# robotseu/ORB_Line_SLAM

Measured on AMD Instinct MI355X. Metric: stereo frames/s extract+match (ORB+LBD), KITTI 1242x375, higher is better.
Workload: dtype u8; 1 GPU; C3: 1242x375 stereo, 2000 ORB + 500 LBD per image, extract + stereo point/line match + f2f LBD match + SearchByBoW vs the previous frame (synthetic k=10 L=6 vocabulary, ComputeBoW included); parallelism=frame-sharded x1, distinct_pairs=512, order=shuffled, scene=default

## Files before the change

### include/orbline.h

```cpp
#ifndef ORBLINE_H
#define ORBLINE_H

#include "orbline_types.h"

#ifdef __cplusplus
extern "C" {
#endif

typedef struct olf_ctx olf_ctx;

const char* olf_last_error(void);
int olf_device_count(void);
int olf_default_params(olf_params* p);

int  olf_ctx_create(const olf_params* p, int width, int height, int max_images, olf_ctx** out);
void olf_ctx_destroy(olf_ctx* ctx);
int  olf_ctx_synchronize(olf_ctx* ctx);
int  olf_ctx_set_input_event(olf_ctx* ctx, void* hip_event);
int  olf_ctx_set_deferred_join(olf_ctx* ctx, int on);
int  olf_stereo_frames_join_dev(olf_ctx* ctx, void* stream);
int  olf_ctx_poll_status(olf_ctx* ctx);

int olf_profile_enable(olf_ctx* ctx, int on);
int olf_profile_reset(olf_ctx* ctx);
// ... 54 lines not shown
int olf_debug_status(olf_ctx* ctx, int32_t* out64);
int olf_debug_status_n(olf_ctx* ctx, int32_t* out, int n);
int olf_debug_lsd_owner(olf_ctx* ctx, int image, uint32_t* out);
int olf_debug_lsd_regions(olf_ctx* ctx, int image, int32_t* start_n, double* angle, int cap, int32_t* count);
int olf_debug_lsd_waves(olf_ctx* ctx, int waves_per_image, int rob_entries);
int olf_debug_lsd_groups(olf_ctx* ctx, int groups);
int olf_debug_lsd_scatter(olf_ctx* ctx, int on);
int olf_debug_lsd_log_cap(olf_ctx* ctx, int entries);
int olf_debug_seed_sort(olf_ctx* ctx, const uint32_t* keys, int n, int kthr, int depth_limit, uint32_t* out, int32_t* out_n);
int olf_debug_seed_sort_mode(olf_ctx* ctx, int mode);
int olf_debug_seed_sort_wide(olf_ctx* ctx, const uint64_t* keys, int n, int64_t kthr, int depth_limit, int full, uint32_t* out, int32_t* out_n);
int olf_debug_lsd_pool(olf_ctx* ctx, int pool_chunks);
int olf_debug_fdiv_sweep(olf_ctx* ctx, uint64_t seed, int blocks, int per_thread, uint64_t* mismatches);
int olf_debug_sqrtq_sweep(olf_ctx* ctx, int count, uint64_t* mismatches);
int olf_debug_align_sweep(olf_ctx* ctx, uint64_t seed, int blocks, int per_thread, uint64_t* out3);

int olf_stereo_points_dev(olf_ctx* ctx, int n_pairs, const olf_keypoint* d_kps, const uint8_t* d_desc, const int32_t* d_counts,
                          float* d_uright, float* d_depth, void* stream);
int olf_stereo_points(olf_ctx* ctx, const uint8_t* images, int n_pairs, olf_keypoint* kps, uint8_t* desc, int32_t* counts,
                      float* uright, float* depth);

int olf_match_bf_dev(olf_ctx* ctx, const uint8_t* d_descA, const int32_t* d_nA, int strideA, int a_step, const uint8_t* d_descB,
                     const int32_t* d_nB, int strideB, int b_step, int n_sets, float nnr, int best_lr, int32_t* d_m12, void* stream);
int olf_match_bf(olf_ctx* ctx, const uint8_t* descA, int nA, const uint8_t* descB, int nB, float nnr, int best_lr, int32_t* m12);
int olf_knn2(olf_ctx* ctx, const uint8_t* descQ, int nQ, const uint8_t* descT, int nT, int32_t* idx0, int32_t* dist0, int32_t* dist1);
int olf_match_candidates_dev(olf_ctx* ctx, const uint8_t* d_descQ, int nQ, const uint8_t* d_descT, int nT, const int32_t* d_cand_offsets,
                             const int32_t* d_cand_idx, uint16_t* d_dist, void* stream);
int olf_match_candidates(olf_ctx* ctx, const uint8_t* descQ, int nQ, const uint8_t* descT, int nT, const int32_t* cand_offsets,
                         const int32_t* cand_idx, uint16_t* dist);
typedef struct olf_frame_view {
// ... 149 lines not shown
```

### orb_line_slam_amd/_lib.py

```python
import ctypes as C
import os
import numpy as np

_HERE = os.path.dirname(os.path.abspath(__file__))
LIB_PATH = os.environ.get("OLF_LIB_PATH", os.path.join(_HERE, "csrc", "liborbline_hip.so"))
SYNTH_PATH = os.path.join(_HERE, "csrc", "libolf_synth.so")

OLF_OK, OLF_ERR_INVALID, OLF_ERR_CAPACITY, OLF_ERR_HIP, OLF_ERR_NODEVICE = 0, -1, -2, -3, -4
DESC_BYTES = 32

KEYPOINT_DTYPE = np.dtype([("x", "<f4"), ("y", "<f4"), ("size", "<f4"), ("angle", "<f4"), ("response", "<f4"),
                           ("octave", "<i4"), ("class_id", "<i4")])
KEYLINE_DTYPE = np.dtype([("angle", "<f4"), ("class_id", "<i4"), ("octave", "<i4"), ("pt_x", "<f4"), ("pt_y", "<f4"),
                          ("response", "<f4"), ("size", "<f4"), ("startPointX", "<f4"), ("startPointY", "<f4"),
                          ("endPointX", "<f4"), ("endPointY", "<f4"), ("sPointInOctaveX", "<f4"),
                          ("sPointInOctaveY", "<f4"), ("ePointInOctaveX", "<f4"), ("ePointInOctaveY", "<f4"),
                          ("lineLength", "<f4"), ("numOfPixels", "<i4")])
assert KEYPOINT_DTYPE.itemsize == 28 and KEYLINE_DTYPE.itemsize == 68


class OrbParams(C.Structure):
    _fields_ = [("nfeatures", C.c_int32), ("scale_factor", C.c_float), ("nlevels", C.c_int32),
                ("ini_th_fast", C.c_int32), ("min_th_fast", C.c_int32), ("conv_gauss_sum256", C.c_int32)]

# ... 144 lines not shown
        L.olf_ctx_set_input_event.argtypes = [C.c_void_p, C.c_void_p]
        L.olf_ctx_set_deferred_join.argtypes = [C.c_void_p, C.c_int]
        L.olf_stereo_frames_join_dev.argtypes = [C.c_void_p, C.c_void_p]
        L.olf_stereo_points_mask_dev.argtypes = [C.c_void_p, C.c_void_p, C.c_size_t, C.c_void_p, C.c_void_p]
        L.olf_search_by_projection_batch_dev.argtypes = [C.c_void_p, C.POINTER(TrackBatchC), C.c_int, C.c_float, C.c_void_p, C.c_int, C.c_int,
                                                         C.c_void_p, C.c_void_p, C.c_void_p, C.c_void_p]
        L.olf_unproject_stereo_dev.argtypes = [C.c_void_p, C.c_int, C.c_int, C.c_void_p, C.c_void_p, C.c_void_p] + [C.c_float] * 4 + [C.c_void_p] * 3
        L.olf_predict_scale_thresholds.argtypes = [C.c_void_p, C.c_int, C.c_void_p]
        L.olf_is_in_frustum_batch_dev.argtypes = [C.c_void_p, C.POINTER(TrackBatchC), C.c_int, C.POINTER(LocalMapC), C.c_void_p, C.c_float] + [C.c_void_p] * 5
        L.olf_search_local_map_batch_dev.argtypes = [C.c_void_p, C.POINTER(TrackBatchC), C.c_int, C.POINTER(LocalMapC), C.c_void_p, C.c_float, C.c_float,
                                                     C.c_void_p, C.c_float, C.c_void_p, C.c_void_p, C.c_void_p]
        L.olf_debug_copy_bandwidth.argtypes =[C.c_void_p, C.c_size_t, C.c_int, C.POINTER(C.c_double)]
        L.olf_debug_fdiv_sweep.argtypes = [C.c_void_p, C.c_uint64, C.c_int, C.c_int, C.POINTER(C.c_uint64)]
        L.olf_debug_sqrtq_sweep.argtypes = [C.c_void_p, C.c_int, C.POINTER(C.c_uint64)]
        L.olf_debug_align_sweep.argtypes = [C.c_void_p, C.c_uint64, C.c_int, C.c_int, C.POINTER(C.c_uint64)]
        L.olf_debug_seed_sort_wide.argtypes = [C.c_void_p, C.c_void_p, C.c_int, C.c_int64, C.c_int, C.c_int, C.c_void_p, C.POINTER(C.c_int32)]
        L.olf_distinctive_descriptors.argtypes = [C.c_void_p, C.c_void_p, C.c_void_p, C.c_int, C.c_void_p]
        L.olf_voc_create.argtypes = [C.c_int, C.c_int, C.c_int, C.c_int, C.c_int, C.c_void_p, C.c_void_p, C.c_void_p, C.c_void_p, C.POINTER(C.c_void_p)]
        L.olf_voc_load_text.argtypes = [C.c_char_p, C.POINTER(C.c_void_p)]
        L.olf_voc_destroy.argtypes = [C.c_void_p]
        L.olf_voc_destroy.restype = None
        L.olf_voc_info.argtypes = [C.c_void_p] + [C.POINTER(C.c_int)] * 6
        L.olf_bow_words_dev.argtypes = [C.c_void_p, C.c_void_p, C.c_void_p, C.c_int, C.c_int, C.c_void_p, C.c_void_p, C.c_void_p, C.c_void_p]
        L.olf_bow_assemble.argtypes = [C.c_void_p, C.c_void_p, C.c_void_p, C.c_void_p, C.c_int, C.c_void_p, C.c_void_p, C.POINTER(C.c_int), C.c_void_p,
                                       C.c_void_p, C.c_void_p, C.POINTER(C.c_int)]
        L.olf_search_by_bow_batch_dev.argtypes = [C.c_void_p, C.c_void_p, C.c_int, C.c_int, C.c_void_p, C.c_void_p, C.c_void_p, C.c_void_p, C.c_void_p, C.c_float, C.c_int, C.c_int, C.c_void_p, C.c_void_p, C.c_void_p]
        L.olf_bow_transform.argtypes = [C.c_void_p, C.c_void_p, C.c_void_p, C.c_int, C.c_int, C.c_void_p, C.c_void_p, C.POINTER(C.c_int), C.c_void_p,
                                        C.c_void_p, C.c_void_p, C.POINTER(C.c_int)]
        L.olf_profile_enable.argtypes = [C.c_void_p, C.c_int]
        L.olf_profile_reset.argtypes = [C.c_void_p]
        L.olf_profile_stage_name.restype = C.c_char_p
        L.olf_profile_stage_name.argtypes = [C.c_int]
        L.olf_profile_read.argtypes = [C.c_void_p, C.c_void_p, C.c_void_p]
        _lib = L
    return _lib


def last_error():
    return lib().olf_last_error().decode()


def device_count():
    return int(lib().olf_device_count())


def default_params():
    p = OlfParams()
    rc = lib().olf_default_params(C.byref(p))
    if rc != OLF_OK:
        raise OlfError(rc, "olf_default_params")
    return p


def check(rc, where):
    if rc != OLF_OK:
        raise OlfError(rc, where)
# ... 51 lines not shown
```

### orb_line_slam_amd/csrc/api.cpp

```cpp
#include "olf_internal.hpp"
#include "line_internal.hpp"
#include "../../include/orbline.h"
#include <map>
#include <mutex>
#include <cstring>
#include <cstddef>

namespace olf {
static thread_local std::string g_err;
void set_error(const std::string& s) { g_err = s; }
}

using namespace olf;

enum { FB_KPS, FB_DESC, FB_COUNTS, FB_URIGHT, FB_DEPTH, FB_KLS, FB_LDESC, FB_LCOUNTS, FB_LMATCHES12, FB_LDISP, FB_LLE, FB_FIELDS };
enum FieldCap { CAP_ONE, CAP_ORB, CAP_LINE };
struct FrameField { const char* name; size_t offset; bool perPair; FieldCap cap; size_t rowBytes; };
#define FIELD(f, perPair, cap, rowBytes) {#f, offsetof(olf_frame_buffers, f), perPair, cap, rowBytes}
constexpr FrameField kFrameFields[] = {
    FIELD(kps, false, CAP_ORB, sizeof(olf_keypoint)),   FIELD(desc, false, CAP_ORB, OLF_DESC_BYTES),    FIELD(counts, false, CAP_ONE, sizeof(int32_t)),
    FIELD(uright, true, CAP_ORB, sizeof(float)),        FIELD(depth, true, CAP_ORB, sizeof(float)),
    FIELD(kls, false, CAP_LINE, sizeof(olf_keyline)),   FIELD(ldesc, false, CAP_LINE, OLF_DESC_BYTES),  FIELD(lcounts, false, CAP_ONE, sizeof(int32_t)),
    FIELD(lmatches12, true, CAP_LINE, sizeof(int32_t)), FIELD(ldisp, true, CAP_LINE, 2 * sizeof(float)), FIELD(lle, true, CAP_LINE, 3 * sizeof(double))};
#undef FIELD
// ... 714 lines not shown
    return OLF_OK;
}

int olf_debug_sqrtq_sweep(olf_ctx* c, int count, uint64_t* mismatches)
{
    if (!c || !mismatches || count < 1) { set_error("olf_debug_sqrtq_sweep: bad argument"); return OLF_ERR_INVALID; }
    void* st = nullptr;
    OLF_TRY(scratch_get(c, 1, 64, &st));
    OLF_HIP_CHECK(hipMemsetAsync(st, 0, 8, c->stream));
    OLF_TRY(launch_sqrtq_sweep(count, (unsigned long long*)st, c->stream));
    OLF_HIP_CHECK(hipMemcpyAsync(mismatches, st, 8, hipMemcpyDeviceToHost, c->stream));
    OLF_HIP_CHECK(hipStreamSynchronize(c->stream));
    return OLF_OK;
}

int olf_debug_align_sweep(olf_ctx* c, uint64_t seed, int blocks, int per_thread, uint64_t* out3)
{
    if (!c || !out3 || blocks < 1 || per_thread < 1) { set_error("olf_debug_align_sweep: bad argument"); return OLF_ERR_INVALID; }
    if (c->line.geom.alignTanLo < 0.f) { set_error("olf_debug_align_sweep: the cheap alignment test is off for lsd_ang_th > 80 degrees"); return OLF_ERR_INVALID; }
    void* st = nullptr;
    OLF_TRY(scratch_get(c, 1, 64, &st));
    OLF_HIP_CHECK(hipMemsetAsync(st, 0, 24, c->stream));
    OLF_TRY(launch_align_sweep(c->lb, (unsigned long long)seed, blocks, per_thread, (unsigned long long*)st, c->stream));
    OLF_HIP_CHECK(hipMemcpyAsync(out3, st, 24, hipMemcpyDeviceToHost, c->stream));
    OLF_HIP_CHECK(hipStreamSynchronize(c->stream));
    return OLF_OK;
}

int olf_orb_debug_candidates(olf_ctx* c, int image, int level, int32_t* xys, int cap, int32_t* count)
{
// ... 475 lines not shown
    if (in_ev) OLF_HIP_CHECK(hipStreamWaitEvent(ls, in_ev, 0));
    else {
        OLF_HIP_CHECK(hipEventRecord(c->ev_fork, s));
        OLF_HIP_CHECK(hipStreamWaitEvent(ls, c->ev_fork, 0));
    }
    if (lg.seedOrder != 1) OLF_HIP_CHECK(hipEventRecord(c->ev_sort, ls));
    {
        StageScope t(c, ls, ST_LSD_FRONT);
        OLF_TRY(launch_lsd_dense(lg, c->lb, plan, d_images, c->W, n_images, ls, false));
        if (lg.seedOrder == 1) OLF_HIP_CHECK(hipEventRecord(c->ev_sort, ls));
        OLF_TRY(launch_lsd_seed_order(lg, c->lb, plan, n_images, ls));
    }
    OLF_HIP_CHECK(hipEventRecord(c->ev_front, ls));
    OLF_TRY(stage_lsd_grow(c, plan, n_images, ls));
    OLF_TRY(stage_lsd_rect(c, plan, n_images, ls));
    OLF_TRY(stage_orb_pyramid(c, d_images, n_images, s));
    OLF_HIP_CHECK(hipStreamWaitEvent(s, c->ev_sort, 0));
    OLF_TRY(stage_orb_blur(c, n_images, s));
    OLF_TRY(launch_lbd_dense(lg, c->lb, d_images, c->W, n_images, s));
    OLF_HIP_CHECK(hipEventRecord(c->ev_lbd, s));
    OLF_HIP_CHECK(hipStreamWaitEvent(s, c->ev_front, 0));
    OLF_TRY(stage_orb_fast(c, n_images, s));
    OLF_TRY(stage_orb_octree(c, n_images, s));
    OLF_TRY(stage_orb_describe(c, n_images, o->kps, o->desc, o->counts, s));
    OLF_HIP_CHECK(hipStreamWaitEvent(ls, c->ev_lbd, 0));
    {
        StageScope t(c, ls, ST_LINE_LBD);
        OLF_TRY(launch_line_select(lg, c->lb, n_images, o->kls, o->lcounts, ls));
        OLF_TRY(launch_lbd_desc(lg, c->lb, n_images, o->kls, o->ldesc, o->lcounts, ls));
    }
    OLF_TRY(stage_stereo_lines(c, n_pairs, o->kls, o->ldesc, o->lcounts, o->lmatches12, o->ldisp, o->lle, ls));
    OLF_HIP_CHECK(hipEventRecord(c->ev_join, ls));
// ... 45 lines not shown
```

### orb_line_slam_amd/csrc/filters.hip

```cpp
#include "olf_internal.hpp"
#include <algorithm>

namespace olf {

constexpr int SF_TW = 128, SF_TH = 32;
constexpr int SF_INW = (SF_TW + 8) / 4;
constexpr int SF_INH = SF_TH + 6;

__device__ __forceinline__ int sf_reflect(int p, int n)
{
    if (p < 0) p = -p;
    if (p >= n) p = 2 * (n - 1) - p;
    return p;
}

__global__ __launch_bounds__(256) void k_sep7(const uint8_t* __restrict__ src, size_t srcImgStride, int srcPitch, uint8_t* __restrict__ dst,
                                              size_t dstImgStride, int dstPitch, int W, int H, Taps7 taps)
{
    __shared__ uint32_t s_in[SF_INH * SF_INW];
    constexpr int HS = (SF_INH + 1) / 2 + ((((SF_INH + 1) / 2) & 1) ? 0 : 1);
    __shared__ uint32_t s_h[SF_TW * HS];
    const int img = blockIdx.z, x0 = blockIdx.x * SF_TW, y0 = blockIdx.y * SF_TH;
    const uint8_t* s = src + (size_t)img * srcImgStride;
    const bool plain = x0 >= 4 && x0 + SF_TW + 4 <= W && y0 >= 3 && y0 + SF_TH + 3 <= H && ((srcPitch | (int)srcImgStride) & 3) == 0 &&
// ... 78 lines not shown

constexpr int SS_ROWS = 16;
constexpr int SS_BROWS = 8;

__device__ __forceinline__ int ss_reflect(int p, int n) { p = p < 0 ? -p : p; return p >= n ? 2 * (n - 1) - p : p; }

template <bool BORDER, int ROWS>
__device__ __forceinline__ void sep7_strip_body(const int t, const uint8_t* __restrict__ src, size_t srcImgStride, int srcPitch, uint8_t* __restrict__ dst,
                                                size_t dstImgStride, int dstPitch, int W, int H, const Taps7& taps, int nsx, int nsy)
{
    const int nb = BORDER ? 1 + ((W + 3) / 4 - (nsx + 1)) : nsx;
    if (t >= nb * nsy) return;
    const int sy = t / nb, si = t - sy * nb;
    const int sx = BORDER ? (si == 0 ? 0 : nsx + si) : si + 1;
    const int x0 = 4 * sx, y0 = sy * ROWS;
    const uint8_t* s = src + (size_t)blockIdx.y * srcImgStride + (x0 - 4);
    uint8_t* d = dst + (size_t)blockIdx.y * dstImgStride + x0;
    const uint32_t tlo = (uint32_t)taps.t[0] | ((uint32_t)taps.t[1] << 8) | ((uint32_t)taps.t[2] << 16) | ((uint32_t)taps.t[3] << 24);
    const uint32_t thi = (uint32_t)taps.t[4] | ((uint32_t)taps.t[5] << 8) | ((uint32_t)taps.t[6] << 16);
    const uint32_t t01 = (uint32_t)taps.t[0] | ((uint32_t)taps.t[1] << 16), t23 = (uint32_t)taps.t[2] | ((uint32_t)taps.t[3] << 16);
    const uint32_t t45 = (uint32_t)taps.t[4] | ((uint32_t)taps.t[5] << 16), t6lo = (uint32_t)taps.t[6], t6hi = (uint32_t)taps.t[6] << 16;
    typedef unsigned short us2 __attribute__((ext_vector_type(2)));
    auto dot2 = [](uint32_t a, uint32_t b, uint32_t c) -> uint32_t {
        us2 va, vb;
        __builtin_memcpy(&va, &a, 4); __builtin_memcpy(&vb, &b, 4);
        return __builtin_amdgcn_udot2(va, vb, c, false);
    };
    struct Raw { uint32_t w[3]; };
    auto load_row = [&](int y) -> Raw {
        Raw r;
        const uint8_t* row = s + (size_t)ss_reflect(min(y, H + 2), H) * srcPitch;
        if (!BORDER) __builtin_memcpy(r.w, row, 12);
        else {
#pragma unroll
            for (int k = 0; k < 3; ++k) {
                uint32_t v = 0;
#pragma unroll
                for (int b = 0; b < 4; ++b) {
                    const int x = x0 - 4 + 4 * k + b;
                    v |= (uint32_t)row[ss_reflect(min(x, W + 2), W) - (x0 - 4)] << (8 * b);
                }
                r.w[k] = v;
            }
        }
        return r;
    };
    auto hrow = [&](const Raw& r, uint32_t* o) {
        const uint32_t* w = r.w;
        o[0] = __builtin_amdgcn_udot4(__builtin_amdgcn_alignbyte(w[2], w[1], 1u), thi, __builtin_amdgcn_udot4(__builtin_amdgcn_alignbyte(w[1], w[0], 1u), tlo, 0u, false), false);
        o[1] = __builtin_amdgcn_udot4(__builtin_amdgcn_alignbyte(w[2], w[1], 2u), thi, __builtin_amdgcn_udot4(__builtin_amdgcn_alignbyte(w[1], w[0], 2u), tlo, 0u, false), false);
        o[2] = __builtin_amdgcn_udot4(__builtin_amdgcn_alignbyte(w[2], w[1], 3u), thi, __builtin_amdgcn_udot4(__builtin_amdgcn_alignbyte(w[1], w[0], 3u), tlo, 0u, false), false);
        o[3] = __builtin_amdgcn_udot4(w[2], thi, __builtin_amdgcn_udot4(w[1], tlo, 0u, false), false);
    };
    auto pair = [&](const Raw& ra, const Raw& rb, uint32_t* Pj) {
        uint32_t a[4], b[4];
        hrow(ra, a); hrow(rb, b);
#pragma unroll
        for (int c = 0; c < 4; ++c) Pj[c] = a[c] | (b[c] << 16);
    };
    uint32_t P[ROWS / 2 + 3][4];
    Raw nx[4];
    {
        Raw r0 = load_row(y0 - 3), r1 = load_row(y0 - 2), r2 = load_row(y0 - 1), r3 = load_row(y0), r4 = load_row(y0 + 1), r5 = load_row(y0 + 2);
#pragma unroll
        for (int k = 0; k < 4; ++k) nx[k] = load_row(y0 + 3 + k);
        pair(r0, r1, P[0]); pair(r2, r3, P[1]); pair(r4, r5, P[2]);
    }
#pragma unroll
    for (int g = 0; g < ROWS / 4; ++g) {
        const Raw c0 = nx[0], c1 = nx[1], c2 = nx[2], c3 = nx[3];
        if (g + 1 < ROWS / 4) {
#pragma unroll
            for (int k = 0; k < 4; ++k) nx[k] = load_row(y0 + 4 * (g + 1) + 3 + k);
            __builtin_amdgcn_sched_barrier(0);
        }
        pair(c0, c1, P[2 * g + 3]); pair(c2, c3, P[2 * g + 4]);
        uint32_t res[4][4];
#pragma unroll
        for (int c = 0; c < 4; ++c) {
            const uint32_t D0 = P[2 * g][c], D1 = P[2 * g + 1][c], D2 = P[2 * g + 2][c], D3 = P[2 * g + 3][c], D4 = P[2 * g + 4][c];
            const uint32_t E0 = __builtin_amdgcn_alignbyte(D1, D0, 2u), E1 = __builtin_amdgcn_alignbyte(D2, D1, 2u);
            const uint32_t E2 = __builtin_amdgcn_alignbyte(D3, D2, 2u), E3 = __builtin_amdgcn_alignbyte(D4, D3, 2u);
            res[0][c] = dot2(D3, t6lo, dot2(D2, t45, dot2(D1, t23, dot2(D0, t01, 32768u))));
            res[1][c] = dot2(D3, t6hi, dot2(E2, t45, dot2(E1, t23, dot2(E0, t01, 32768u))));
            res[2][c] = dot2(D4, t6lo, dot2(D3, t45, dot2(D2, t23, dot2(D1, t01, 32768u))));
            res[3][c] = dot2(D4, t6hi, dot2(E3, t45, dot2(E2, t23, dot2(E1, t01, 32768u))));
        }
#pragma unroll
        for (int rr = 0; rr < 4; ++rr) {
            const int gy = y0 + 4 * g + rr;
            if (gy < H) {
                const uint32_t a0 = min(res[rr][0] >> 16, 255u), a1 = min(res[rr][1] >> 16, 255u), a2 = min(res[rr][2] >> 16, 255u), a3 = min(res[rr][3] >> 16, 255u);
                const uint32_t v = a0 | (a1 << 8) | (a2 << 16) | (a3 << 24);
                if (!BORDER) __builtin_memcpy(d + (size_t)gy * dstPitch, &v, 4);
                else {
#pragma unroll
                    for (int b = 0; b < 4; ++b) if (x0 + b < W) d[(size_t)gy * dstPitch + b] = (uint8_t)(v >> (8 * b));
                }
            }
        }
    }
}

template <bool BORDER>
__global__ __launch_bounds__(256) void k_sep7_strip(const uint8_t* __restrict__ src, size_t srcImgStride, int srcPitch, uint8_t* __restrict__ dst,
                                                    size_t dstImgStride, int dstPitch, int W, int H, Taps7 taps, int nsx, int nsy)
{
    sep7_strip_body<BORDER, BORDER ? SS_BROWS : SS_ROWS>(blockIdx.x * 256 + threadIdx.x, src, srcImgStride, srcPitch, dst, dstImgStride, dstPitch, W, H, taps, nsx, nsy);
}

int launch_sep7(const uint8_t* src, size_t srcImgStride, int srcPitch, uint8_t* dst, size_t dstImgStride, int dstPitch, int W, int H,
                const int* taps7, int n_images, hipStream_t s)
{
    Taps7 t;
    for (int i = 0; i < 7; ++i) t.t[i] = taps7[i];
    if (t.t[3] == 256) {
        for (int i = 0; i < n_images; ++i)
            OLF_HIP_CHECK(hipMemcpy2DAsync(dst + (size_t)i * dstImgStride, dstPitch, src + (size_t)i * srcImgStride, srcPitch, W, H, hipMemcpyDeviceToDevice, s));
        return OLF_OK;
    }
    for (int i = 0; i < 7; ++i)
        if (t.t[i] < 0 || t.t[i] > 255) { set_error("launch_sep7: taps must be 8-bit fractions"); return OLF_ERR_INVALID; }
    if (W >= 16 && H >= 8 && (dstPitch & 3) == 0 && (dstImgStride & 3) == 0 && (reinterpret_cast<uintptr_t>(dst) & 3) == 0) {
        const int nsx = (W - 7) / 4, nsy = (H + SS_ROWS - 1) / SS_ROWS, nb = 1 + ((W + 3) / 4 - (nsx + 1));
        const int nsyB = (H + SS_BROWS - 1) / SS_BROWS;
        hipLaunchKernelGGL(k_sep7_strip<false>, dim3((nsx * nsy + 255) / 256, n_images), dim3(256), 0, s, src, srcImgStride, srcPitch, dst, dstImgStride, dstPitch, W, H, t, nsx, nsy);
        hipLaunchKernelGGL(k_sep7_strip<true>, dim3((nb * nsyB + 255) / 256, n_images), dim3(256), 0, s, src, srcImgStride, srcPitch, dst, dstImgStride, dstPitch, W, H, t, nsx, nsyB);
        OLF_HIP_CHECK(hipGetLastError());
        return OLF_OK;
    }
    hipLaunchKernelGGL(k_sep7, dim3((W + SF_TW - 1) / SF_TW, (H + SF_TH - 1) / SF_TH, n_images), dim3(256), 0, s, src, srcImgStride, srcPitch,
                       dst, dstImgStride, dstPitch, W, H, t);
    OLF_HIP_CHECK(hipGetLastError());
    return OLF_OK;
}

struct TapsWide { int r; int t[15]; };
__global__ __launch_bounds__(256) void k_sep_wide(const uint8_t* __restrict__ src, size_t srcImgStride, int srcPitch, uint8_t* __restrict__ dst,
// ... 202 lines not shown
{
    strip = strip && (dstPitch & 3) == 0 && (dstImgStride & 3) == 0 && srcPitch >= 8;
    if (strip) {
        const int nsx = (dw + 3) / 4;
        hipLaunchKernelGGL(k_resize_strip, dim3((nsx + 63) / 64, (dh + RS_ROWS - 1) / RS_ROWS, n_images), dim3(64), 0, s, src, srcImgStride, srcPitch, sw, sh,
                           dst, dstImgStride, dstPitch, dw, dh, d_rx, d_ry, nsx);
        OLF_HIP_CHECK(hipGetLastError());
        return OLF_OK;
    }
    hipLaunchKernelGGL(k_resize_tiled, dim3((dw + RZ_TW - 1) / RZ_TW, (dh + RZ_TH - 1) / RZ_TH, n_images), dim3(256), 0, s, src, srcImgStride,
                       srcPitch, sw, sh, dst, dstImgStride, dstPitch, dw, dh, d_rx, d_ry);
    OLF_HIP_CHECK(hipGetLastError());
    return OLF_OK;
}

}
```

### orb_line_slam_amd/csrc/lbd.hip

```cpp
#include "line_internal.hpp"
#include "device_math.hpp"

namespace olf {

#define OLF_TRY_RC(expr) do { int _rc = (expr); if (_rc != OLF_OK) return _rc; } while (0)

__constant__ int8_t c_bandPairs[64] = {
#include "lbd_band_pairs.inc"
};

constexpr int LS_LDS_KEYS = 4096;

template <typename P>
__device__ __forceinline__ void ls_bitonic_desc(P sk, int sortN, int tid)
{
    for (int k = 2; k <= sortN; k <<= 1)
        for (int j = k >> 1; j > 0; j >>= 1) {
            for (int i = tid; i < sortN; i += 256) {
                const int ixj = i ^ j;
                if (ixj > i) {
                    const unsigned long long a = sk[i], b = sk[ixj];
                    const bool desc = (i & k) == 0;
                    if (desc ? (a < b) : (a > b)) { sk[i] = b; sk[ixj] = a; }
                }
// ... 303 lines not shown
int launch_lbd_desc(const LineGeom& g, const LineDeviceBufs& b, int n_images, const olf_keyline* d_kls, uint8_t* d_desc, const int* d_counts, hipStream_t s)
{
    hipLaunchKernelGGL(k_lbd_prep, dim3((g.outCap + 63) / 64, n_images), dim3(64), 0, s, b.geom, d_kls, d_counts, reinterpret_cast<float2*>(b.lbdStarts));
    if (g.W + 256 < 32768 && g.H + 256 < 32768)
        hipLaunchKernelGGL(k_lbd_rows<true>, dim3((g.outCap + 3) / 4, n_images), dim3(256), 0, s, b.geom, b.dxdy, d_kls, d_counts,
                           reinterpret_cast<const float2*>(b.lbdStarts), reinterpret_cast<float4*>(b.rowSums));
    else
        hipLaunchKernelGGL(k_lbd_rows<false>, dim3((g.outCap + 3) / 4, n_images), dim3(256), 0, s, b.geom, b.dxdy, d_kls, d_counts,
                           reinterpret_cast<const float2*>(b.lbdStarts), reinterpret_cast<float4*>(b.rowSums));
    hipLaunchKernelGGL(k_lbd_desc, dim3((g.outCap + 63) / 64, n_images), dim3(64), 0, s, b.geom, reinterpret_cast<const float4*>(b.rowSums),
                       d_counts, d_desc);
    OLF_HIP_CHECK(hipGetLastError());
    return OLF_OK;
}

}
```

### orb_line_slam_amd/csrc/lsd_seedsort.hip

```cpp
#include "lsd_device.hpp"
#pragma clang diagnostic ignored "-Winline-asm"

namespace olf {

constexpr int SS_TOP_MIN = 8192, SS_TOP_JOBS = 128, SS_TOP_LEVELS = 8, SS_TOP_FINAL = 512;
constexpr int SS_JW = 12;
constexpr int SS_TOP_WORDS = 8 + 2 * SS_TOP_JOBS * SS_JW + SS_TOP_FINAL * 5;
constexpr int SS_CAP = 1024;
constexpr int SS_NE_MEM = 4;
constexpr int SS_NE_LDS = 2;

struct SsCtx {
    uint32_t* A;
    uint32_t* sbuf;
    uint32_t* out;
    int ldsFirst;
    int lane;
};

__device__ __forceinline__ uint32_t ssK(uint32_t e) { return e >> 22; }
__device__ __forceinline__ int ssU(int v) { return __builtin_amdgcn_readfirstlane(v); }
template <bool LDS> __device__ __forceinline__ uint32_t ss_ld(const SsCtx& c, int i) { return LDS ? c.sbuf[i - c.ldsFirst] : c.A[i]; }
template <bool LDS> __device__ __forceinline__ void ss_st(const SsCtx& c, int i, uint32_t v) { if (LDS) c.sbuf[i - c.ldsFirst] = v; else c.A[i] = v; }
__device__ __forceinline__ void ss_async_ld(const uint32_t* g, unsigned lds_byte_off)
// ... 488 lines not shown
#undef SS_PUSH
#undef SS_LOCK
#undef SS_UNLOCK
#ifdef OLF_SS_PROF
    SSPROF(SP_OTHER);
    if (NW == 1 && lane == 0 && img == 0) { long long* o = reinterpret_cast<long long*>(status + 16); for (int q = 0; q < SP_N; ++q) o[q] = sp_acc[q]; }
#endif
    if (NW == 1) { if (lane == 0) keyCount[img * 32] = listedEnd; }
    else {
        if (lane == 0) atomicMax(&ctl[3], listedEnd);
        __syncthreads();
        if (threadIdx.x == 0) { if (Gs > 1 && topImg) atomicMax(&keyCount[img * 32], ctl[3]); else keyCount[img * 32] = ctl[3]; }
    }
}

__global__ __launch_bounds__(64) void k_lsd_seedsort(const LineGeom* __restrict__ gp, uint32_t* keysInAll, uint32_t* keysOutAll, int* __restrict__ keyCount,
                                                     const int* __restrict__ maxN, int* __restrict__ status, int nOverride, int kthrOverride, int depthOverride)
{
    __shared__ __align__(8) uint32_t s_buf[SS_CAP];
    __shared__ __align__(8) uint32_t s_x[4 * 64 * SS_NE_LDS];
    static_assert(4 * 64 * SS_NE_MEM <= SS_CAP && 2 * 64 * SS_NE_MEM <= 4 * 64 * SS_NE_LDS, "memory path: queues in the range buffer, staged blocks in s_x");
    ss_sort_image<1, SS_NE_MEM>(*gp, blockIdx.x, gridDim.x, keysInAll, keysOutAll, keyCount, maxN, status, nOverride, kthrOverride, depthOverride, s_buf, s_x, nullptr);
}

template <int NW, int NEM>
__global__ __launch_bounds__(64 * NW) void k_lsd_seedsort_mw(const LineGeom* __restrict__ gp, uint32_t* keysInAll, uint32_t* keysOutAll, int* __restrict__ keyCount,
                                                            const int* __restrict__ maxN, int* __restrict__ status, int nOverride, int kthrOverride, int depthOverride,
                                                            int n_images, int* __restrict__ topAll, int Gs)
{
    extern __shared__ __align__(8) uint32_t s_dyn[];
    constexpr int BUFW = 4 * 64 * NEM, XW = 2 * 64 * NEM;
    const int blk = (int)blockIdx.x / Gs, grp = (int)blockIdx.x % Gs;
    static_assert(XW >= 4 * 64 * SS_NE_LDS, "the LDS path's queues fit the staging area");
    const int wv = threadIdx.x >> 6;
    uint32_t* s_x = s_dyn + (size_t)wv * XW;
    uint32_t* s_buf = s_dyn + (size_t)NW * XW + (size_t)wv * BUFW;
// ... 292 lines not shown
    }
    if (p.sortTop) { const int rc = launch_seedsort_top(g, b, n_images, s, nOverride, kthrOverride, depthOverride); if (rc != OLF_OK) return rc; }
    if (p.sortGroups > 1 && nOverride >= 0) OLF_HIP_CHECK(hipMemsetAsync(b.keyCount, 0, (size_t)n_images * 32 * sizeof(int), s));
    hipLaunchKernelGGL((k_lsd_seedsort_mw<NW, NEM>), dim3(n_images * p.sortGroups), dim3(64 * NW), lds, s, b.geom, b.keysA, b.keysB, b.keyCount, b.maxN, b.status,
                       nOverride, kthrOverride, depthOverride, n_images, p.sortTop ? b.topBuf : (int*)nullptr, p.sortGroups);
    return OLF_OK;
}

int launch_lsd_seedsort(const LineGeom& g, const LineDeviceBufs& b, const LsdPlan& p, int n_images, hipStream_t s, int nOverride, int kthrOverride, int depthOverride)
{
    int rc = OLF_OK;
    if (p.sortWaves == 4) rc = launch_seedsort_mw<4, 8>(g, b, p, n_images, s, nOverride, kthrOverride, depthOverride);
    else if (p.sortWaves == 8) rc = launch_seedsort_mw<8, 8>(g, b, p, n_images, s, nOverride, kthrOverride, depthOverride);
    else if (p.sortWaves == 2) rc = launch_seedsort_mw<2, 8>(g, b, p, n_images, s, nOverride, kthrOverride, depthOverride);
    else
        hipLaunchKernelGGL(k_lsd_seedsort, dim3(n_images), dim3(64), 0, s, b.geom, b.keysA, b.keysB, b.keyCount, b.maxN, b.status, nOverride, kthrOverride, depthOverride);
    if (rc != OLF_OK) return rc;
    OLF_HIP_CHECK(hipGetLastError());
    return OLF_OK;
}

}
```

### orb_line_slam_amd/csrc/olf_internal.hpp

```cpp
#pragma once
#include <hip/hip_runtime.h>
#include <stdint.h>
#include <string>
#include <vector>
#include "../../include/orbline_types.h"

#define OLF_HIP_CHECK(expr)                                                                 \
    do {                                                                                    \
        hipError_t _e = (expr);                                                             \
        if (_e != hipSuccess) {                                                             \
            olf::set_error(std::string(#expr) + ": " + hipGetErrorString(_e));              \
            return OLF_ERR_HIP;                                                             \
        }                                                                                   \
    } while (0)

struct olf_ctx;

namespace olf {

void set_error(const std::string& s);

hipStream_t ctx_stream(olf_ctx* c);
int ctx_scratch(olf_ctx* c, int slot, size_t bytes, void** out);
int* ctx_status(olf_ctx* c);
// ... 91 lines not shown
    ResizeCoef* rx = nullptr;
    ResizeCoef* ry = nullptr;
    OrbGeom* geom = nullptr;
    int* status = nullptr;
    unsigned char* octSpill = nullptr;
};

int launch_orb_pyramid(const OrbGeom& g, const OrbDeviceBufs& b, const uint8_t* d_in, int n_images, hipStream_t s);
int launch_orb_fast(const OrbGeom& g, const OrbDeviceBufs& b, int n_images, hipStream_t s);
int launch_orb_octree(const OrbGeom& g, const OrbDeviceBufs& b, int n_images, hipStream_t s);
size_t octree_lds_bytes(int M);
int launch_orb_blur(const OrbGeom& g, const OrbDeviceBufs& b, int n_images, hipStream_t s);
int launch_orb_describe(const OrbGeom& g, const OrbDeviceBufs& b, int n_images, olf_keypoint* d_kps, uint8_t* d_desc,
                        int* d_counts, int out_cap, hipStream_t s);

struct Taps7 { int t[7]; };
int launch_sep7(const uint8_t* src, size_t srcImgStride, int srcPitch, uint8_t* dst, size_t dstImgStride, int dstPitch, int W, int H,
                const int* taps7, int n_images, hipStream_t s);
int launch_sep_wide(const uint8_t* src, size_t srcImgStride, int srcPitch, uint8_t* dst, size_t dstImgStride, int dstPitch, int W, int H,
                    const int* taps, int r, int n_images, hipStream_t s);

bool resize_tiled_fits(const ResizeCoef* rx, const ResizeCoef* ry, int sw, int sh, int dw, int dh);
bool resize_strip_fits(const ResizeCoef* rx, int sw, int dw, int ncols = 4);
int launch_resize_tiled(const uint8_t* src, size_t srcImgStride, int srcPitch, int sw, int sh, uint8_t* dst, size_t dstImgStride, int dstPitch,
                        int dw, int dh, const ResizeCoef* d_rx, const ResizeCoef* d_ry, int n_images, hipStream_t s, bool strip = false);

int launch_cvt_gray(const uint8_t* src, uint8_t* dst, int w, int h, int code, int n_images, hipStream_t s);
int launch_init_rectify_map(const double* ir9, const double* k8, double fx, double fy, double u0, double v0, int w, int h, float* d_map1, float* d_map2,
                            hipStream_t s);
int launch_remap_linear(const uint8_t* src, int sw, int sh, const float* mapx, const float* mapy, int dw, int dh, uint8_t* dst, int n_images,
// ... 23 lines not shown
```

### orb_line_slam_amd/csrc/orb_pyramid.hip

```cpp
#include "olf_internal.hpp"

namespace olf {

__global__ __launch_bounds__(256) void k_ingest(const uint8_t* __restrict__ in, uint8_t* __restrict__ pyr,
                                                int W, int H, int in_pitch, int pitch0, int pyrBytes)
{
    const int img = blockIdx.y;
    const int segs = (W + 15) >> 4;
    const int idx = blockIdx.x * 256 + threadIdx.x;
    if (idx >= segs * H) return;
    const int y = idx / segs, x = (idx - y * segs) * 16;
    const uint8_t* src = in + (size_t)img * H * in_pitch + (size_t)y * in_pitch + x;
    uint4 v = make_uint4(0u, 0u, 0u, 0u);
    if (x + 16 <= W) __builtin_memcpy(&v, src, 16);
    else {
        uint32_t w[4] = {0u, 0u, 0u, 0u};
#pragma unroll
        for (int k = 0; k < 16; ++k)
            if (x + k < W) w[k >> 2] |= (uint32_t)src[k] << (8 * (k & 3));
        v = make_uint4(w[0], w[1], w[2], w[3]);
    }
    *reinterpret_cast<uint4*>(pyr + (size_t)img * pyrBytes + (size_t)y * pitch0 + x) = v;
}

// ... 290 lines not shown
    OLF_HIP_CHECK(hipGetLastError());
    return OLF_OK;
}

int launch_orb_blur(const OrbGeom& g, const OrbDeviceBufs& b, int n_images, hipStream_t s)
{
    for (int l = 0; l < g.nlevels; ++l) {
        const LevelGeom& L = g.lv[l];
        int rc = launch_sep7(b.pyr + L.offset, (size_t)g.pyrBytes, L.pitch, b.blur + L.offset, (size_t)g.pyrBytes, L.pitch, L.w, L.h, g.blurTaps,
                             n_images, s);
        if (rc != OLF_OK) return rc;
    }
    return OLF_OK;
}

}
```

Baseline: 14920 stereo frames/s.

## Cut register pressure in sep7 border path and seedsort, reorder ORB pyramid wait

The border variant of the separable 7-tap blur now precomputes reflected column offsets once per thread, loads rows in pairs separated by scheduling barriers, and uses 32-bit offsets with wide stores where possible. Both the blur and the single-wave seed sort kernel are pinned to 8 waves per EU, and the seed sort moves its LDS to a dynamic allocation. The ORB pyramid launch now waits for the LSD sort event first, which changes how the two streams overlap. Debug entry points for kernel attributes and a standalone sep7 are added to check register and scratch use and to verify the output.

```diff
diff --git a/include/orbline.h b/include/orbline.h
--- a/include/orbline.h
+++ b/include/orbline.h
@@ -92,6 +92,8 @@
 int olf_debug_fdiv_sweep(olf_ctx* ctx, uint64_t seed, int blocks, int per_thread, uint64_t* mismatches);
 int olf_debug_sqrtq_sweep(olf_ctx* ctx, int count, uint64_t* mismatches);
 int olf_debug_align_sweep(olf_ctx* ctx, uint64_t seed, int blocks, int per_thread, uint64_t* out3);
+int olf_debug_kernel_attributes(const char* kernel, int32_t* num_regs, int32_t* shared_bytes, int32_t* local_bytes);
+int olf_debug_sep7(const uint8_t* images, int width, int height, int n_images, const int32_t* taps7, uint8_t* out);
 
 int olf_stereo_points_dev(olf_ctx* ctx, int n_pairs, const olf_keypoint* d_kps, const uint8_t* d_desc, const int32_t* d_counts,
                           float* d_uright, float* d_depth, void* stream);
diff --git a/orb_line_slam_amd/_lib.py b/orb_line_slam_amd/_lib.py
--- a/orb_line_slam_amd/_lib.py
+++ b/orb_line_slam_amd/_lib.py
@@ -182,6 +182,8 @@
         L.olf_debug_fdiv_sweep.argtypes = [C.c_void_p, C.c_uint64, C.c_int, C.c_int, C.POINTER(C.c_uint64)]
         L.olf_debug_sqrtq_sweep.argtypes = [C.c_void_p, C.c_int, C.POINTER(C.c_uint64)]
         L.olf_debug_align_sweep.argtypes = [C.c_void_p, C.c_uint64, C.c_int, C.c_int, C.POINTER(C.c_uint64)]
+        L.olf_debug_kernel_attributes.argtypes = [C.c_char_p] + [C.POINTER(C.c_int32)] * 3
+        L.olf_debug_sep7.argtypes = [C.c_void_p, C.c_int, C.c_int, C.c_int, C.c_void_p, C.c_void_p]
         L.olf_debug_seed_sort_wide.argtypes = [C.c_void_p, C.c_void_p, C.c_int, C.c_int64, C.c_int, C.c_int, C.c_void_p, C.POINTER(C.c_int32)]
         L.olf_distinctive_descriptors.argtypes = [C.c_void_p, C.c_void_p, C.c_void_p, C.c_int, C.c_void_p]
         L.olf_voc_create.argtypes = [C.c_int, C.c_int, C.c_int, C.c_int, C.c_int, C.c_void_p, C.c_void_p, C.c_void_p, C.c_void_p, C.POINTER(C.c_void_p)]
@@ -208,6 +210,22 @@
     return lib().olf_last_error().decode()
 
 
+def kernel_attributes(name):
+    regs, lds, scratch = C.c_int32(), C.c_int32(), C.c_int32()
+    check(lib().olf_debug_kernel_attributes(name.encode(), C.byref(regs), C.byref(lds), C.byref(scratch)), "olf_debug_kernel_attributes")
+    return regs.value, lds.value, scratch.value
+
+
+def sep7(images, taps7):
+    images = np.ascontiguousarray(images, np.uint8)
+    taps = np.ascontiguousarray(taps7, np.int32)
+    assert images.ndim == 3 and taps.shape == (7,)
+    out = np.zeros_like(images)
+    n, h, w = images.shape
+    check(lib().olf_debug_sep7(ptr(images), w, h, n, ptr(taps), ptr(out)), "olf_debug_sep7")
+    return out
+
+
 def device_count():
     return int(lib().olf_device_count())
 
diff --git a/orb_line_slam_amd/csrc/api.cpp b/orb_line_slam_amd/csrc/api.cpp
--- a/orb_line_slam_amd/csrc/api.cpp
+++ b/orb_line_slam_amd/csrc/api.cpp
@@ -752,6 +752,40 @@
     return OLF_OK;
 }
 
+int olf_debug_kernel_attributes(const char* kernel, int32_t* num_regs, int32_t* shared_bytes, int32_t* local_bytes)
+{
+    if (!kernel || !num_regs || !shared_bytes || !local_bytes) { set_error("olf_debug_kernel_attributes: null argument"); return OLF_ERR_INVALID; }
+    const void* fn = nullptr;
+    for (const void* f : {filters_kernel(kernel), orb_pyramid_kernel(kernel), lbd_kernel(kernel), seedsort_kernel(kernel)})
+        if (f) fn = f;
+    if (!fn) { set_error(std::string("olf_debug_kernel_attributes: no kernel named ") + kernel); return OLF_ERR_INVALID; }
+    hipFuncAttributes a;
+    OLF_HIP_CHECK(hipFuncGetAttributes(&a, fn));
+    *num_regs = a.numRegs; *shared_bytes = (int32_t)a.sharedSizeBytes; *local_bytes = (int32_t)a.localSizeBytes;
+    return OLF_OK;
+}
+
+int olf_debug_sep7(const uint8_t* images, int width, int height, int n_images, const int32_t* taps7, uint8_t* out)
+{
+    if (!images || !taps7 || !out || width < 1 || height < 1 || n_images < 1) { set_error("olf_debug_sep7: bad argument"); return OLF_ERR_INVALID; }
+    const int pitch = (width + 3) & ~3;
+    const size_t stride = (size_t)pitch * height, bytes = stride * n_images;
+    uint8_t *d_src = nullptr, *d_dst = nullptr;
+    int taps[7];
+    for (int i = 0; i < 7; ++i) taps[i] = taps7[i];
+    int rc = OLF_ERR_HIP;
+    if (hipMalloc(&d_src, bytes) == hipSuccess && hipMalloc(&d_dst, bytes) == hipSuccess &&
+        hipMemcpy2D(d_src, pitch, images, width, width, (size_t)height * n_images, hipMemcpyHostToDevice) == hipSuccess &&
+        hipMemset(d_dst, 0, bytes) == hipSuccess) {
+        rc = launch_sep7(d_src, stride, pitch, d_dst, stride, pitch, width, height, taps, n_images, nullptr);
+        if (rc == OLF_OK && (hipDeviceSynchronize() != hipSuccess ||
+                             hipMemcpy2D(out, width, d_dst, pitch, width, (size_t)height * n_images, hipMemcpyDeviceToHost) != hipSuccess)) rc = OLF_ERR_HIP;
+    }
+    if (rc == OLF_ERR_HIP) set_error(std::string("olf_debug_sep7: ") + hipGetErrorString(hipGetLastError()));
+    (void)hipFree(d_src); (void)hipFree(d_dst);
+    return rc;
+}
+
 int olf_debug_align_sweep(olf_ctx* c, uint64_t seed, int blocks, int per_thread, uint64_t* out3)
 {
     if (!c || !out3 || blocks < 1 || per_thread < 1) { set_error("olf_debug_align_sweep: bad argument"); return OLF_ERR_INVALID; }
@@ -1257,8 +1291,8 @@
     OLF_HIP_CHECK(hipEventRecord(c->ev_front, ls));
     OLF_TRY(stage_lsd_grow(c, plan, n_images, ls));
     OLF_TRY(stage_lsd_rect(c, plan, n_images, ls));
+    OLF_HIP_CHECK(hipStreamWaitEvent(s, c->ev_sort, 0));
     OLF_TRY(stage_orb_pyramid(c, d_images, n_images, s));
-    OLF_HIP_CHECK(hipStreamWaitEvent(s, c->ev_sort, 0));
     OLF_TRY(stage_orb_blur(c, n_images, s));
     OLF_TRY(launch_lbd_dense(lg, c->lb, d_images, c->W, n_images, s));
     OLF_HIP_CHECK(hipEventRecord(c->ev_lbd, s));
diff --git a/orb_line_slam_amd/csrc/filters.hip b/orb_line_slam_amd/csrc/filters.hip
--- a/orb_line_slam_amd/csrc/filters.hip
+++ b/orb_line_slam_amd/csrc/filters.hip
@@ -116,8 +116,9 @@
     const int sy = t / nb, si = t - sy * nb;
     const int sx = BORDER ? (si == 0 ? 0 : nsx + si) : si + 1;
     const int x0 = 4 * sx, y0 = sy * ROWS;
-    const uint8_t* s = src + (size_t)blockIdx.y * srcImgStride + (x0 - 4);
-    uint8_t* d = dst + (size_t)blockIdx.y * dstImgStride + x0;
+    const int ncol = W - x0;
+    const uint8_t* s = src + (size_t)blockIdx.y * srcImgStride;
+    uint8_t* d = dst + (size_t)blockIdx.y * dstImgStride;
     const uint32_t tlo = (uint32_t)taps.t[0] | ((uint32_t)taps.t[1] << 8) | ((uint32_t)taps.t[2] << 16) | ((uint32_t)taps.t[3] << 24);
     const uint32_t thi = (uint32_t)taps.t[4] | ((uint32_t)taps.t[5] << 8) | ((uint32_t)taps.t[6] << 16);
     const uint32_t t01 = (uint32_t)taps.t[0] | ((uint32_t)taps.t[1] << 16), t23 = (uint32_t)taps.t[2] | ((uint32_t)taps.t[3] << 16);
@@ -128,22 +129,21 @@
         __builtin_memcpy(&va, &a, 4); __builtin_memcpy(&vb, &b, 4);
         return __builtin_amdgcn_udot2(va, vb, c, false);
     };
+    uint32_t xp[5];
+    if (BORDER) {
+#pragma unroll
+        for (int k = 0; k < 5; ++k)
+            xp[k] = (uint32_t)ss_reflect(min(x0 - 3 + 2 * k, W + 2), W) | ((uint32_t)ss_reflect(min(x0 - 2 + 2 * k, W + 2), W) << 16);
+    }
     struct Raw { uint32_t w[3]; };
     auto load_row = [&](int y) -> Raw {
         Raw r;
-        const uint8_t* row = s + (size_t)ss_reflect(min(y, H + 2), H) * srcPitch;
-        if (!BORDER) __builtin_memcpy(r.w, row, 12);
+        const uint32_t row = (uint32_t)(ss_reflect(min(y, H + 2), H) * srcPitch);
+        if (!BORDER) __builtin_memcpy(r.w, s + (row + (uint32_t)(x0 - 4)), 12);
         else {
-#pragma unroll
-            for (int k = 0; k < 3; ++k) {
-                uint32_t v = 0;
-#pragma unroll
-                for (int b = 0; b < 4; ++b) {
-                    const int x = x0 - 4 + 4 * k + b;
-                    v |= (uint32_t)row[ss_reflect(min(x, W + 2), W) - (x0 - 4)] << (8 * b);
-                }
-                r.w[k] = v;
-            }
+            r.w[0] = r.w[1] = r.w[2] = 0;
+#pragma unroll
+            for (int k = 0; k < 10; ++k) r.w[(k + 1) >> 2] |= (uint32_t)s[row + ((k & 1) ? xp[k >> 1] >> 16 : xp[k >> 1] & 0xffffu)] << (8 * ((k + 1) & 3));
         }
         return r;
     };
@@ -160,23 +160,40 @@
 #pragma unroll
         for (int c = 0; c < 4; ++c) Pj[c] = a[c] | (b[c] << 16);
     };
+    auto pair_at = [&](int y, uint32_t* Pj) {
+        uint32_t a[4], b[4];
+        { const Raw r = load_row(y); hrow(r, a); }
+        __builtin_amdgcn_sched_barrier(0);
+        { const Raw r = load_row(y + 1); hrow(r, b); }
+        __builtin_amdgcn_sched_barrier(0);
+#pragma unroll
+        for (int c = 0; c < 4; ++c) Pj[c] = a[c] | (b[c] << 16);
+    };
     uint32_t P[ROWS / 2 + 3][4];
     Raw nx[4];
-    {
+    if (!BORDER) {
         Raw r0 = load_row(y0 - 3), r1 = load_row(y0 - 2), r2 = load_row(y0 - 1), r3 = load_row(y0), r4 = load_row(y0 + 1), r5 = load_row(y0 + 2);
 #pragma unroll
         for (int k = 0; k < 4; ++k) nx[k] = load_row(y0 + 3 + k);
         pair(r0, r1, P[0]); pair(r2, r3, P[1]); pair(r4, r5, P[2]);
+    } else {
+#pragma unroll
+        for (int j = 0; j < 3; ++j) pair_at(y0 - 3 + 2 * j, P[j]);
     }
 #pragma unroll
     for (int g = 0; g < ROWS / 4; ++g) {
-        const Raw c0 = nx[0], c1 = nx[1], c2 = nx[2], c3 = nx[3];
-        if (g + 1 < ROWS / 4) {
-#pragma unroll
-            for (int k = 0; k < 4; ++k) nx[k] = load_row(y0 + 4 * (g + 1) + 3 + k);
-            __builtin_amdgcn_sched_barrier(0);
-        }
-        pair(c0, c1, P[2 * g + 3]); pair(c2, c3, P[2 * g + 4]);
+        if (!BORDER) {
+            const Raw c0 = nx[0], c1 = nx[1], c2 = nx[2], c3 = nx[3];
+            if (g + 1 < ROWS / 4) {
+#pragma unroll
+                for (int k = 0; k < 4; ++k) nx[k] = load_row(y0 + 4 * (g + 1) + 3 + k);
+                __builtin_amdgcn_sched_barrier(0);
+            }
+            pair(c0, c1, P[2 * g + 3]); pair(c2, c3, P[2 * g + 4]);
+        } else {
+#pragma unroll
+            for (int j = 3; j < 5; ++j) pair_at(y0 + 4 * g - 3 + 2 * j, P[2 * g + j]);
+        }
         uint32_t res[4][4];
 #pragma unroll
         for (int c = 0; c < 4; ++c) {
@@ -193,11 +210,13 @@
             const int gy = y0 + 4 * g + rr;
             if (gy < H) {
                 const uint32_t a0 = min(res[rr][0] >> 16, 255u), a1 = min(res[rr][1] >> 16, 255u), a2 = min(res[rr][2] >> 16, 255u), a3 = min(res[rr][3] >> 16, 255u);
-                const uint32_t v = a0 | (a1 << 8) | (a2 << 16) | (a3 << 24);
-                if (!BORDER) __builtin_memcpy(d + (size_t)gy * dstPitch, &v, 4);
+                uint32_t v = a0 | (a1 << 8) | (a2 << 16) | (a3 << 24);
+                if (BORDER) asm volatile("" : "+v"(v));
+                const uint32_t o = (uint32_t)(gy * dstPitch + x0);
+                if (!BORDER || ncol > 3) __builtin_memcpy(d + o, &v, 4);
                 else {
 #pragma unroll
-                    for (int b = 0; b < 4; ++b) if (x0 + b < W) d[(size_t)gy * dstPitch + b] = (uint8_t)(v >> (8 * b));
+                    for (int b = 0; b < 4; ++b) if (b < ncol) d[o + b] = (uint8_t)(v >> (8 * b));
                 }
             }
         }
@@ -205,8 +224,9 @@
 }
 
 template <bool BORDER>
-__global__ __launch_bounds__(256) void k_sep7_strip(const uint8_t* __restrict__ src, size_t srcImgStride, int srcPitch, uint8_t* __restrict__ dst,
-                                                    size_t dstImgStride, int dstPitch, int W, int H, Taps7 taps, int nsx, int nsy)
+__global__ __launch_bounds__(256) __attribute__((amdgpu_waves_per_eu(8, 8)))
+void k_sep7_strip(const uint8_t* __restrict__ src, size_t srcImgStride, int srcPitch, uint8_t* __restrict__ dst, size_t dstImgStride, int dstPitch, int W, int H,
+                  Taps7 taps, int nsx, int nsy)
 {
     sep7_strip_body<BORDER, BORDER ? SS_BROWS : SS_ROWS>(blockIdx.x * 256 + threadIdx.x, src, srcImgStride, srcPitch, dst, dstImgStride, dstPitch, W, H, taps, nsx, nsy);
 }
@@ -223,7 +243,7 @@
     }
     for (int i = 0; i < 7; ++i)
         if (t.t[i] < 0 || t.t[i] > 255) { set_error("launch_sep7: taps must be 8-bit fractions"); return OLF_ERR_INVALID; }
-    if (W >= 16 && H >= 8 && (dstPitch & 3) == 0 && (dstImgStride & 3) == 0 && (reinterpret_cast<uintptr_t>(dst) & 3) == 0) {
+    if (W >= 16 && W < 65536 && H >= 8 && (dstPitch & 3) == 0 && (dstImgStride & 3) == 0 && (reinterpret_cast<uintptr_t>(dst) & 3) == 0) {
         const int nsx = (W - 7) / 4, nsy = (H + SS_ROWS - 1) / SS_ROWS, nb = 1 + ((W + 3) / 4 - (nsx + 1));
         const int nsyB = (H + SS_BROWS - 1) / SS_BROWS;
         hipLaunchKernelGGL(k_sep7_strip<false>, dim3((nsx * nsy + 255) / 256, n_images), dim3(256), 0, s, src, srcImgStride, srcPitch, dst, dstImgStride, dstPitch, W, H, t, nsx, nsy);
@@ -456,4 +476,13 @@
     return OLF_OK;
 }
 
-}
+const void* filters_kernel(const char* name)
+{
+    const std::string n(name);
+    if (n == "k_sep7_strip<false>") return reinterpret_cast<const void*>(&k_sep7_strip<false>);
+    if (n == "k_sep7_strip<true>") return reinterpret_cast<const void*>(&k_sep7_strip<true>);
+    if (n == "k_resize_strip") return reinterpret_cast<const void*>(&k_resize_strip);
+    return nullptr;
+}
+
+}
diff --git a/orb_line_slam_amd/csrc/lbd.hip b/orb_line_slam_amd/csrc/lbd.hip
--- a/orb_line_slam_amd/csrc/lbd.hip
+++ b/orb_line_slam_amd/csrc/lbd.hip
@@ -341,4 +341,6 @@
     return OLF_OK;
 }
 
-}
+const void* lbd_kernel(const char* name) { return std::string(name) == "k_sobel3" ? reinterpret_cast<const void*>(&k_sobel3) : nullptr; }
+
+}
diff --git a/orb_line_slam_amd/csrc/lsd_seedsort.hip b/orb_line_slam_amd/csrc/lsd_seedsort.hip
--- a/orb_line_slam_amd/csrc/lsd_seedsort.hip
+++ b/orb_line_slam_amd/csrc/lsd_seedsort.hip
@@ -526,12 +526,16 @@
     }
 }
 
-__global__ __launch_bounds__(64) void k_lsd_seedsort(const LineGeom* __restrict__ gp, uint32_t* keysInAll, uint32_t* keysOutAll, int* __restrict__ keyCount,
-                                                     const int* __restrict__ maxN, int* __restrict__ status, int nOverride, int kthrOverride, int depthOverride)
-{
-    __shared__ __align__(8) uint32_t s_buf[SS_CAP];
-    __shared__ __align__(8) uint32_t s_x[4 * 64 * SS_NE_LDS];
+constexpr int SS_SORT_LDS_BYTES = (SS_CAP + 4 * 64 * SS_NE_LDS) * 4;
+__global__ __launch_bounds__(64) __attribute__((amdgpu_waves_per_eu(8, 8)))
+void k_lsd_seedsort(const LineGeom* __restrict__ gp, uint32_t* keysInAll, uint32_t* keysOutAll, int* __restrict__ keyCount,
+                    const int* __restrict__ maxN, int* __restrict__ status, int nOverride, int kthrOverride, int depthOverride)
+{
+    extern __shared__ __align__(8) uint32_t s_sort[];
+    uint32_t* const s_buf = s_sort;
+    uint32_t* const s_x = s_sort + SS_CAP;
     static_assert(4 * 64 * SS_NE_MEM <= SS_CAP && 2 * 64 * SS_NE_MEM <= 4 * 64 * SS_NE_LDS, "memory path: queues in the range buffer, staged blocks in s_x");
+    static_assert(SS_SORT_LDS_BYTES == 6144, "24 agents per CU");
     ss_sort_image<1, SS_NE_MEM>(*gp, blockIdx.x, gridDim.x, keysInAll, keysOutAll, keyCount, maxN, status, nOverride, kthrOverride, depthOverride, s_buf, s_x, nullptr);
 }
 
@@ -854,10 +858,12 @@
     else if (p.sortWaves == 8) rc = launch_seedsort_mw<8, 8>(g, b, p, n_images, s, nOverride, kthrOverride, depthOverride);
     else if (p.sortWaves == 2) rc = launch_seedsort_mw<2, 8>(g, b, p, n_images, s, nOverride, kthrOverride, depthOverride);
     else
-        hipLaunchKernelGGL(k_lsd_seedsort, dim3(n_images), dim3(64), 0, s, b.geom, b.keysA, b.keysB, b.keyCount, b.maxN, b.status, nOverride, kthrOverride, depthOverride);
+        hipLaunchKernelGGL(k_lsd_seedsort, dim3(n_images), dim3(64), SS_SORT_LDS_BYTES, s, b.geom, b.keysA, b.keysB, b.keyCount, b.maxN, b.status, nOverride, kthrOverride, depthOverride);
     if (rc != OLF_OK) return rc;
     OLF_HIP_CHECK(hipGetLastError());
     return OLF_OK;
 }
 
-}
+const void* seedsort_kernel(const char* name) { return std::string(name) == "k_lsd_seedsort" ? reinterpret_cast<const void*>(&k_lsd_seedsort) : nullptr; }
+
+}
diff --git a/orb_line_slam_amd/csrc/olf_internal.hpp b/orb_line_slam_amd/csrc/olf_internal.hpp
--- a/orb_line_slam_amd/csrc/olf_internal.hpp
+++ b/orb_line_slam_amd/csrc/olf_internal.hpp
@@ -129,6 +129,11 @@
 int launch_orb_describe(const OrbGeom& g, const OrbDeviceBufs& b, int n_images, olf_keypoint* d_kps, uint8_t* d_desc,
                         int* d_counts, int out_cap, hipStream_t s);
 
+const void* filters_kernel(const char* name);
+const void* orb_pyramid_kernel(const char* name);
+const void* lbd_kernel(const char* name);
+const void* seedsort_kernel(const char* name);
+
 struct Taps7 { int t[7]; };
 int launch_sep7(const uint8_t* src, size_t srcImgStride, int srcPitch, uint8_t* dst, size_t dstImgStride, int dstPitch, int W, int H,
                 const int* taps7, int n_images, hipStream_t s);
diff --git a/orb_line_slam_amd/csrc/orb_pyramid.hip b/orb_line_slam_amd/csrc/orb_pyramid.hip
--- a/orb_line_slam_amd/csrc/orb_pyramid.hip
+++ b/orb_line_slam_amd/csrc/orb_pyramid.hip
@@ -328,4 +328,6 @@
     return OLF_OK;
 }
 
-}
+const void* orb_pyramid_kernel(const char* name) { return std::string(name) == "k_ingest" ? reinterpret_cast<const void*>(&k_ingest) : nullptr; }
+
+}
```

New measurement: 15210 stereo frames/s (median of 4 runs). No clear change (+1.9%).
